# thomaspingel/neilpy

Hardware: AMD Instinct MI355X
Metric: Mcells/s through SMRF progressive_filter, 16384x16384 fp32 DEM (higher is better)
Workload: dtype f32

## Files before the change

### neilpy_amd/csrc/ero_inc_adopt.inc

```
inline constexpr unsigned char kEroIncAdoptF32[65] = {
    0, 0, 0, 0, 0, 0, 0, 0, 0, 0, 0, 0, 0, 0, 0, 0, 0,
    0, 0, 0, 0, 1, 0, 0, 0, 0, 0, 0, 1, 1, 0, 1, 0, 0,
    0, 0, 1, 0, 1, 0, 1, 1, 1, 1, 1, 1, 1, 1, 1, 1, 1,
    0, 0, 0, 0, 0, 0, 0, 0, 0, 0, 0, 0, 0, 0};
```

### neilpy_amd/csrc/morph_incero.h

```cpp
#pragma once
#include "morph_ring.h"

namespace smrf {

#include "ero_inc.inc"
#include "ero_inc_adopt.inc"

#define SMRF_INCERO_MIN_RADIUS 16
#define SMRF_INCERO_MAX_RADIUS 64

template <typename T>
struct IncEroArgs {
  const T* e_prev;
  const T* last;
  T* out;
  int rows, cols;
  long long ld;
  int seg;
  int nt;
  int plain_tiles;
};

template <int R>
struct IncEroCfg {
  static constexpr int N = kEroInc[R].n;
  static constexpr int DY = kEroInc[R].reach;
  static constexpr int TW = 256, NP = 4, ROWS = 2 * NP;
  static constexpr int W = TW + 2 * DY;
  static constexpr int NPOS = (W + TW - 1) / TW;
  static constexpr int NACC = 2 * DY + ROWS;
  static constexpr int G = 4;
  static constexpr int NJ = NP * N;
  static constexpr int NG = (NJ + G - 1) / G;
  static constexpr int gsize(int g) { const int n = NJ - g * G; return n < 0 ? 0 : n > G ? G : n; }
  static constexpr int dy(int k) { return kEroInc[R].p[k].dy; }
  static constexpr int dx(int k) { return kEroInc[R].p[k].dx; }
  static constexpr int slot(int j) { return 2 * (j / N) - dy(j % N) + DY; }
  struct Plan { short seq[NJ > 0 ? NJ : 1], first[NACC]; };
  static constexpr Plan make_plan() {
    Plan pl{};
    int n = 0;
    for (int s = 0; s < NACC; ++s) {
      pl.first[s] = NJ;
      for (int j = 0; j < NJ; ++j)
        if (slot(j) == s) pl.seq[n++] = (short)j;
    }
    for (int i = NJ - 1; i >= 0; --i) pl.first[slot(pl.seq[i])] = pl.first[slot(pl.seq[i]) + 1] = (short)i;
    return pl;
  }
  static constexpr Plan plan = make_plan();
  static constexpr bool plan_ok() {
    int seen[NJ > 0 ? NJ : 1] = {};
    for (int i = 0; i < NJ; ++i) ++seen[plan.seq[i]];
    for (int j = 0; j < NJ; ++j)
      if (seen[j] != 1) return false;
    for (int s = 0; s < NACC; ++s) {
      int firsts = 0, touches = 0;
      for (int i = 0; i < NJ; ++i)
        for (int h = 0; h < 2; ++h)
          if (slot(plan.seq[i]) + h == s) { ++touches; firsts += plan.first[s] == i; }
      if (firsts != (touches > 0)) return false;
      if (s + ROWS < NACC && plan.first[s] < NJ && plan.first[s + ROWS] < NJ && plan.first[s] >= plan.first[s + ROWS]) return false;
    }
    return true;
  }
  static constexpr int DELTA = (ROWS - (2 * DY) % ROWS) % ROWS;
  static constexpr int LDS_CELLS = N > 0 ? 2 * NP * W : 1;
};

template <typename T, int R>
__global__ __launch_bounds__(256) void inc_erode_kernel(const IncEroArgs<T> a) {
  using C = IncEroCfg<R>;
  using T2 = typename Vec2<T>::type;
  constexpr int N = C::N, DY = C::DY, TW = C::TW, NP = C::NP, ROWS = C::ROWS, W = C::W, NPOS = C::NPOS, NACC = C::NACC, G = C::G;
  __shared__ T2 L[C::LDS_CELLS];
  const int tid = threadIdx.x;
  int bx, by;
  smrf_xcd_tile(a.plain_tiles, [] { return true; }, bx, by);
  const int x0 = bx * TW, x = x0 + tid;
  const int ys = by * a.seg, ye = min(a.rows, ys + a.seg);
  if (ys >= ye) return;
  const int xc = x < a.cols ? x : a.cols - 1;
  const int xl = smrf_fold(xc - 1, a.cols), xr = smrf_fold(xc + 1, a.cols);
  int cpos[NPOS];
  bool act[NPOS];
#pragma unroll
  for (int i = 0; i < NPOS; ++i) {
    act[i] = tid + i * TW < W;
    cpos[i] = smrf_fold(x0 - DY + tid + (act[i] ? i * TW : 0), a.cols);
  }
  T acc[NACC];
#pragma unroll
  for (int i = 0; i < NACC; ++i) acc[i] = ident<T>(false);

  static_assert(C::plan_ok(), "the batch plan");
  int o0 = ys - 2 * DY - C::DELTA;
  const int nb = (ye - o0 + ROWS - 1) / ROWS;
  RowFold rf(o0 + DY, a.rows);
  T2 pf[NP][NPOS];
  auto prefetch = [&]() {
#pragma unroll
    for (int p = 0; p < NP; ++p) {
      const T* ra = a.last + (long long)rf.at(2 * p) * a.ld;
      const T* rb = a.last + (long long)rf.at(2 * p + 1) * a.ld;
#pragma unroll
      for (int i = 0; i < NPOS; ++i)
        { pf[p][i].x = ra[cpos[i]]; pf[p][i].y = rb[cpos[i]]; }
    }
    rf.advance(ROWS);
  };
  if constexpr (N > 0) prefetch();

  T outv[ROWS];
  auto store_rows = [&](int ob) {
#pragma unroll
    for (int j = 0; j < ROWS; ++j)
      if (ob + j < ye && x < a.cols) smrf_store_out(a.out + (long long)(ob + j) * a.ld + x, outv[j], a.nt);
  };
  for (int b = 0; b < nb; ++b, o0 += ROWS) {
    const unsigned lds_b = (unsigned)(size_t)(__attribute__((address_space(3))) void*)(L + (b & 1) * NP * W + tid);
    if constexpr (N > 0) {
#pragma unroll
      for (int p = 0; p < NP; ++p)
#pragma unroll
        for (int i = 0; i < NPOS; ++i)
          lds_write2(lds_b + (unsigned)((p * W + (i < NPOS - 1 || act[i] ? i * TW : 0)) * (int)sizeof(T2)), pf[p][i]);
      lds_wait<0>();
      __syncthreads();
    }
    if (o0 - ROWS >= ys) store_rows(o0 - ROWS);
    const bool store = o0 >= ys;
    T ec[ROWS + 2], el[ROWS], er[ROWS];
    if (store) {
      RowFold rfe(o0 - 1, a.rows);
#pragma unroll
      for (int j = 0; j < ROWS + 2; ++j) {
        const T* row = a.e_prev + (long long)rfe.at(j) * a.ld;
        ec[j] = row[xc];
        if (j >= 1 && j <= ROWS) { el[j - 1] = row[xl]; er[j - 1] = row[xr]; }
      }
    }
    if constexpr (N > 0) {
      __builtin_amdgcn_sched_barrier(0);
      prefetch();
      __builtin_amdgcn_sched_barrier(0);
      T old[NACC];
#pragma unroll
      for (int s = 0; s < NACC; ++s) old[s] = acc[s];
      [&]<int... S>(std::integer_sequence<int, S...>) {
        (([&] {
           if constexpr (C::plan.first[S] == C::NJ) acc[S] = S + ROWS < NACC ? old[S + ROWS] : ident<T>(false);
         }()),
         ...);
      }(std::make_integer_sequence<int, NACC>{});
      T2 rd[2 * G][2];
      auto issue = [&]<int I>(std::integral_constant<int, I>) {
        constexpr int J = C::plan.seq[I], p = J / N, k = J % N;
        constexpr int offl = (p * W + DY - C::dx(k)) * (int)sizeof(T2), offr = (p * W + DY + C::dx(k)) * (int)sizeof(T2);
        rd[I % (2 * G)][0] = lds_read2<offl>(lds_b, T());
        rd[I % (2 * G)][1] = lds_read2<offr>(lds_b, T());
      };
      auto update = [&]<int S, int I>(std::integral_constant<int, S>, std::integral_constant<int, I>, const T& l, const T& r) {
        static_assert(S >= 0 && S < NACC, "slot outside the ring");
        if constexpr (C::plan.first[S] != I) op3_acc<false>(acc[S], l, r);
        else if constexpr (S + ROWS < NACC) acc[S] = op3<false>(old[S + ROWS], l, r);
        else acc[S] = op2<false>(l, r);
      };
      auto apply = [&]<int I>(std::integral_constant<int, I> i) {
        constexpr int s = C::slot(C::plan.seq[I]);
        update(std::integral_constant<int, s>{}, i, rd[I % (2 * G)][0].x, rd[I % (2 * G)][1].x);
        update(std::integral_constant<int, s + 1>{}, i, rd[I % (2 * G)][0].y, rd[I % (2 * G)][1].y);
      };
      auto issue_group = [&]<int Gi>(std::integral_constant<int, Gi>) {
        [&]<int... I>(std::integer_sequence<int, I...>) {
          (issue(std::integral_constant<int, Gi * G + I>{}), ...);
        }(std::make_integer_sequence<int, C::gsize(Gi)>{});
      };
      auto apply_group = [&]<int Gi>(std::integral_constant<int, Gi>) {
        [&]<int... I>(std::integer_sequence<int, I...>) {
          (apply(std::integral_constant<int, Gi * G + I>{}), ...);
        }(std::make_integer_sequence<int, C::gsize(Gi)>{});
      };
      issue_group(std::integral_constant<int, 0>{});
      [&]<int... Gi>(std::integer_sequence<int, Gi...>) {
        (([&] {
           if constexpr (Gi + 1 < C::NG) {
             issue_group(std::integral_constant<int, Gi + 1>{});
             lds_wait<2 * C::gsize(Gi + 1)>();
           } else {
             lds_wait<0>();
           }
           apply_group(std::integral_constant<int, Gi>{});
         }()),
         ...);
      }(std::make_integer_sequence<int, C::NG>{});
    }
    if (store) {
#pragma unroll
      for (int j = 0; j < ROWS; ++j) {
        T m = op3<false>(ec[j + 1], el[j], er[j]);
        m = op3<false>(m, ec[j], ec[j + 2]);
        if constexpr (N > 0) m = op2<false>(m, acc[j]);
        outv[j] = m;
      }
    }
  }
  if (o0 - ROWS >= ys) store_rows(o0 - ROWS);
}

template <typename T, int R>
int inc_erode_launch(const IncEroArgs<T>& a_in, hipStream_t stream) {
  using C = IncEroCfg<R>;
  constexpr auto kern = inc_erode_kernel<T, R>;
  int resident;
  bool first;
  if (int rc = smrf_resident<kern>(C::TW, 0, resident, first)) return rc;
  if (first && smrf_sw().ring_debug)
    fprintf(stderr, "smrf inc erode: R=%d pairs=%d reach=%d LDS=%zu, %d workgroups/CU resident\n", R, C::N, C::DY,
            C::LDS_CELLS * 2 * sizeof(T), resident);
  IncEroArgs<T> a = a_in;
  const int strips = (a.cols + C::TW - 1) / C::TW;
  a.seg = smrf_seg_len(a.rows, strips, resident, smrf_sw().ring_rounds, 2 * C::DY + C::DELTA, C::ROWS, std::max(32, 4 * C::DY),
                       smrf_sw().seg_rule, a.seg);
  a.plain_tiles = smrf_sw().xcd_remap ? 0 : 1;
  dim3 grid(strips, (a.rows + a.seg - 1) / a.seg);
  hipLaunchKernelGGL(kern, grid, dim3(C::TW), 0, stream, a);
  SMRF_LAUNCH_CHECK();
  return SMRF_OK;
}

}
```

Before: 4132.

## Share LDS reads between mirrored offset pairs in incremental erosion kernel

The incremental erosion kernel now exploits the vertical mirror symmetry of the structuring-element offset table. Each pair of offsets with opposite dy and the same dx reuses one pair of LDS reads to update two accumulator slots, roughly halving LDS read traffic. A compile-time scheduler orders these items so each ring slot's first write follows the right dependency, either splitting pairs or copying old values when no ordering works. Per-radius tables choose the plan kind and whether the cross-shaped neighbourhood global loads move after the LDS phase, and the adoption table enables the incremental path for more radii. The cost is higher compile-time complexity and register pressure from the rescheduled accumulators.

```diff
diff --git a/neilpy_amd/csrc/ero_inc_adopt.inc b/neilpy_amd/csrc/ero_inc_adopt.inc
--- a/neilpy_amd/csrc/ero_inc_adopt.inc
+++ b/neilpy_amd/csrc/ero_inc_adopt.inc
@@ -1,5 +1,5 @@
 inline constexpr unsigned char kEroIncAdoptF32[65] = {
     0, 0, 0, 0, 0, 0, 0, 0, 0, 0, 0, 0, 0, 0, 0, 0, 0,
-    0, 0, 0, 0, 1, 0, 0, 0, 0, 0, 0, 1, 1, 0, 1, 0, 0,
-    0, 0, 1, 0, 1, 0, 1, 1, 1, 1, 1, 1, 1, 1, 1, 1, 1,
+    0, 0, 0, 0, 1, 0, 0, 0, 0, 0, 0, 1, 1, 0, 1, 1, 1,
+    1, 1, 1, 1, 1, 1, 1, 1, 1, 1, 1, 1, 1, 1, 1, 1, 1,
     0, 0, 0, 0, 0, 0, 0, 0, 0, 0, 0, 0, 0, 0};
diff --git a/neilpy_amd/csrc/morph_incero.h b/neilpy_amd/csrc/morph_incero.h
--- a/neilpy_amd/csrc/morph_incero.h
+++ b/neilpy_amd/csrc/morph_incero.h
@@ -8,6 +8,35 @@
 
 #define SMRF_INCERO_MIN_RADIUS 16
 #define SMRF_INCERO_MAX_RADIUS 64
+
+enum { kIncEroPlain = 0, kIncEroMirrorSplit = 1, kIncEroMirrorCopy = 2 };
+inline constexpr unsigned char kIncEroPlanKind[65] = {
+    1, 1, 1, 1, 1, 1, 1, 1, 1, 1, 1, 1, 1, 1, 1, 1, 1,
+    1, 1, 1, 1, 1, 1, 1, 1, 1, 1, 1, 1, 1, 1, 1, 1, 1,
+    1, 1, 1, 1, 1, 1, 1, 1, 1, 1, 2, 2, 1, 1, 1, 1, 1,
+    1, 1, 1, 1, 1, 1, 1, 1, 1, 1, 1, 1, 1, 1};
+inline constexpr unsigned char kIncEroCrossLate[65] = {
+    0, 0, 0, 0, 0, 0, 0, 0, 0, 0, 0, 0, 0, 0, 0, 0, 0,
+    0, 0, 0, 0, 0, 0, 0, 0, 0, 0, 0, 0, 0, 0, 0, 0, 0,
+    0, 0, 0, 0, 0, 1, 0, 0, 0, 0, 1, 1, 0, 0, 0, 1, 1,
+    0, 0, 0, 0, 0, 0, 0, 0, 0, 0, 0, 0, 0, 0};
+#ifndef SMRF_INCERO_MIRROR_GROUP
+#define SMRF_INCERO_MIRROR_GROUP 2
+#endif
+constexpr int inc_ero_plan_kind(int radius) {
+#ifdef SMRF_INCERO_PLAN
+  return SMRF_INCERO_PLAN;
+#else
+  return kIncEroPlanKind[radius];
+#endif
+}
+constexpr bool inc_ero_cross_late(int radius) {
+#ifdef SMRF_INCERO_LATE
+  return SMRF_INCERO_LATE;
+#else
+  return kIncEroCrossLate[radius] != 0;
+#endif
+}
 
 template <typename T>
 struct IncEroArgs {
@@ -29,41 +58,132 @@
   static constexpr int W = TW + 2 * DY;
   static constexpr int NPOS = (W + TW - 1) / TW;
   static constexpr int NACC = 2 * DY + ROWS;
-  static constexpr int G = 4;
+  static constexpr int KIND = N > 0 ? inc_ero_plan_kind(R) : kIncEroPlain;
+  static constexpr int NM = N / 2;
+  static constexpr int G = KIND == kIncEroPlain ? 4 : SMRF_INCERO_MIRROR_GROUP;
   static constexpr int NJ = NP * N;
-  static constexpr int NG = (NJ + G - 1) / G;
-  static constexpr int gsize(int g) { const int n = NJ - g * G; return n < 0 ? 0 : n > G ? G : n; }
   static constexpr int dy(int k) { return kEroInc[R].p[k].dy; }
   static constexpr int dx(int k) { return kEroInc[R].p[k].dx; }
   static constexpr int slot(int j) { return 2 * (j / N) - dy(j % N) + DY; }
-  struct Plan { short seq[NJ > 0 ? NJ : 1], first[NACC]; };
+  static constexpr int mirror(int j) { return (j / N) * N + N - 1 - j % N; }
+  static constexpr bool mirrored() {
+    for (int k = 0; k < N; ++k)
+      if (dy(k) != -dy(N - 1 - k) || dx(k) != dx(N - 1 - k) || dy(k) == 0) return false;
+    return N % 2 == 0;
+  }
+  static constexpr short NONE = 32767;
+  struct Item { short j; bool both; };
+  struct Plan { short n, splits, copies; Item item[NJ > 0 ? NJ : 1]; short first[NACC]; };
   static constexpr Plan make_plan() {
     Plan pl{};
-    int n = 0;
-    for (int s = 0; s < NACC; ++s) {
-      pl.first[s] = NJ;
-      for (int j = 0; j < NJ; ++j)
-        if (slot(j) == s) pl.seq[n++] = (short)j;
-    }
-    for (int i = NJ - 1; i >= 0; --i) pl.first[slot(pl.seq[i])] = pl.first[slot(pl.seq[i]) + 1] = (short)i;
+    for (int s = 0; s < NACC; ++s) pl.first[s] = NONE;
+    auto emit = [&](int j, bool both) {
+      for (int h = 0; h < (both ? 2 : 1); ++h)
+        for (int b = 0; b < 2; ++b) {
+          short& f = pl.first[slot(h ? mirror(j) : j) + b];
+          if (f == NONE) f = pl.n;
+        }
+      pl.item[pl.n++] = Item{(short)j, both};
+    };
+    if constexpr (KIND == kIncEroPlain) {
+      for (int s = 0; s < NACC; ++s)
+        for (int j = 0; j < NJ; ++j)
+          if (slot(j) == s) emit(j, false);
+    } else {
+      constexpr int NGR = NP * NM;
+      auto jlo = [](int g) { return (g / NM) * N + NM + g % NM; };
+      auto lo = [&](int g) { return slot(jlo(g)); };
+      auto hi = [&](int g) { return slot(mirror(jlo(g))); };
+      bool touched[NACC] = {}, done[NACC] = {};
+      unsigned char state[NGR > 0 ? NGR : 1] = {};
+      for (int g = 0; g < NGR; ++g) touched[lo(g)] = touched[lo(g) + 1] = touched[hi(g)] = touched[hi(g) + 1] = true;
+      auto unready = [&](int g, int part) {
+        int u = 0;
+        for (int h = 0; h < 2; ++h)
+          if (part >> h & 1)
+            for (int b = 0; b < 2; ++b) {
+              const int t = (h ? hi(g) : lo(g)) + b;
+              u += !(done[t] || t < ROWS || !touched[t - ROWS] || done[t - ROWS]);
+            }
+        return u;
+      };
+      auto run = [&](int g, int part) {
+        pl.copies += (short)unready(g, part);
+        if (part & 1) done[lo(g)] = done[lo(g) + 1] = true;
+        if (part & 2) done[hi(g)] = done[hi(g) + 1] = true;
+        state[g] |= (unsigned char)part;
+        emit(part == 2 ? mirror(jlo(g)) : jlo(g), part == 3);
+      };
+      for (int left = 2 * NGR; left > 0;) {
+        int bg = -1, bpart = 0, bkey = 0;
+        for (int g = 0; g < NGR; ++g) {
+          const int part = 3 & ~state[g];
+          if (!part || unready(g, part)) continue;
+          const int key = part & 1 ? lo(g) : hi(g);
+          if (bg < 0 || key < bkey) bg = g, bpart = part, bkey = key;
+        }
+        if (bg < 0 && KIND == kIncEroMirrorSplit) {
+          int bcnt = -1;
+          for (int g = 0; g < NGR; ++g)
+            for (int part = 1; part <= 2 && !state[g]; ++part) {
+              if (unready(g, part)) continue;
+              const int s = part == 1 ? lo(g) : hi(g);
+              const bool was[2] = {done[s], done[s + 1]};
+              done[s] = done[s + 1] = true;
+              state[g] |= (unsigned char)part;
+              int cnt = 0;
+              for (int h = 0; h < NGR; ++h) {
+                const int rest = 3 & ~state[h];
+                const int a = lo(h) - s - ROWS, c = hi(h) - s - ROWS;
+                if (rest && ((a >= -1 && a <= 1) || (c >= -1 && c <= 1)) && !unready(h, rest)) ++cnt;
+              }
+              state[g] = 0;
+              done[s] = was[0], done[s + 1] = was[1];
+              if (cnt > bcnt || (cnt == bcnt && s < bkey)) bg = g, bpart = part, bkey = s, bcnt = cnt;
+            }
+          ++pl.splits;
+        } else if (bg < 0) {
+          int bu = 0;
+          for (int g = 0; g < NGR; ++g) {
+            if (state[g]) continue;
+            const int u = unready(g, 3);
+            if (bg < 0 || u < bu || (u == bu && lo(g) < bkey)) bg = g, bpart = 3, bkey = lo(g), bu = u;
+          }
+        }
+        run(bg, bpart);
+        left -= bpart == 3 ? 2 : 1;
+      }
+    }
     return pl;
   }
   static constexpr Plan plan = make_plan();
+  static constexpr int NI = plan.n;
+  static constexpr int NG = (NI + G - 1) / G;
+  static constexpr int gsize(int g) { const int n = NI - g * G; return n < 0 ? 0 : n > G ? G : n; }
   static constexpr bool plan_ok() {
+    if (N > 0 && !mirrored()) return false;
     int seen[NJ > 0 ? NJ : 1] = {};
-    for (int i = 0; i < NJ; ++i) ++seen[plan.seq[i]];
+    for (int i = 0; i < NI; ++i) {
+      ++seen[plan.item[i].j];
+      if (plan.item[i].both) ++seen[mirror(plan.item[i].j)];
+    }
     for (int j = 0; j < NJ; ++j)
       if (seen[j] != 1) return false;
+    if (KIND == kIncEroPlain ? NI != NJ || plan.splits || plan.copies : NI != NP * NM + plan.splits) return false;
+    if ((KIND == kIncEroMirrorSplit && plan.copies) || (KIND == kIncEroMirrorCopy && plan.splits)) return false;
+    int late = 0;
     for (int s = 0; s < NACC; ++s) {
-      int firsts = 0, touches = 0;
-      for (int i = 0; i < NJ; ++i)
-        for (int h = 0; h < 2; ++h)
-          if (slot(plan.seq[i]) + h == s) { ++touches; firsts += plan.first[s] == i; }
-      if (firsts != (touches > 0)) return false;
-      if (s + ROWS < NACC && plan.first[s] < NJ && plan.first[s + ROWS] < NJ && plan.first[s] >= plan.first[s + ROWS]) return false;
-    }
-    return true;
-  }
+      int earliest = NONE, touches = 0;
+      for (int i = NI - 1; i >= 0; --i)
+        for (int h = 0; h < (plan.item[i].both ? 2 : 1); ++h)
+          for (int b = 0; b < 2; ++b)
+            if (slot(h ? mirror(plan.item[i].j) : plan.item[i].j) + b == s) { ++touches; earliest = i; }
+      if (plan.first[s] != earliest) return false;
+      if (touches && s + ROWS < NACC && plan.first[s + ROWS] != NONE && plan.first[s] >= plan.first[s + ROWS]) ++late;
+    }
+    return late == plan.copies;
+  }
+  static constexpr bool LATE = N > 0 && inc_ero_cross_late(R);
   static constexpr int DELTA = (ROWS - (2 * DY) % ROWS) % ROWS;
   static constexpr int LDS_CELLS = N > 0 ? 2 * NP * W : 1;
 };
@@ -131,7 +251,7 @@
     if (o0 - ROWS >= ys) store_rows(o0 - ROWS);
     const bool store = o0 >= ys;
     T ec[ROWS + 2], el[ROWS], er[ROWS];
-    if (store) {
+    auto cross_loads = [&]() {
       RowFold rfe(o0 - 1, a.rows);
 #pragma unroll
       for (int j = 0; j < ROWS + 2; ++j) {
@@ -139,7 +259,9 @@
         ec[j] = row[xc];
         if (j >= 1 && j <= ROWS) { el[j - 1] = row[xl]; er[j - 1] = row[xr]; }
       }
-    }
+    };
+    if constexpr (!C::LATE)
+      if (store) cross_loads();
     if constexpr (N > 0) {
       __builtin_amdgcn_sched_barrier(0);
       prefetch();
@@ -149,13 +271,13 @@
       for (int s = 0; s < NACC; ++s) old[s] = acc[s];
       [&]<int... S>(std::integer_sequence<int, S...>) {
         (([&] {
-           if constexpr (C::plan.first[S] == C::NJ) acc[S] = S + ROWS < NACC ? old[S + ROWS] : ident<T>(false);
+           if constexpr (C::plan.first[S] == C::NONE) acc[S] = S + ROWS < NACC ? old[S + ROWS] : ident<T>(false);
          }()),
          ...);
       }(std::make_integer_sequence<int, NACC>{});
       T2 rd[2 * G][2];
       auto issue = [&]<int I>(std::integral_constant<int, I>) {
-        constexpr int J = C::plan.seq[I], p = J / N, k = J % N;
+        constexpr int J = C::plan.item[I].j, p = J / N, k = J % N;
         constexpr int offl = (p * W + DY - C::dx(k)) * (int)sizeof(T2), offr = (p * W + DY + C::dx(k)) * (int)sizeof(T2);
         rd[I % (2 * G)][0] = lds_read2<offl>(lds_b, T());
         rd[I % (2 * G)][1] = lds_read2<offr>(lds_b, T());
@@ -167,9 +289,11 @@
         else acc[S] = op2<false>(l, r);
       };
       auto apply = [&]<int I>(std::integral_constant<int, I> i) {
-        constexpr int s = C::slot(C::plan.seq[I]);
+        constexpr int s = C::slot(C::plan.item[I].j), m = C::slot(C::mirror(C::plan.item[I].j));
         update(std::integral_constant<int, s>{}, i, rd[I % (2 * G)][0].x, rd[I % (2 * G)][1].x);
+        if constexpr (C::plan.item[I].both) update(std::integral_constant<int, m>{}, i, rd[I % (2 * G)][0].x, rd[I % (2 * G)][1].x);
         update(std::integral_constant<int, s + 1>{}, i, rd[I % (2 * G)][0].y, rd[I % (2 * G)][1].y);
+        if constexpr (C::plan.item[I].both) update(std::integral_constant<int, m + 1>{}, i, rd[I % (2 * G)][0].y, rd[I % (2 * G)][1].y);
       };
       auto issue_group = [&]<int Gi>(std::integral_constant<int, Gi>) {
         [&]<int... I>(std::integer_sequence<int, I...>) {
@@ -196,6 +320,7 @@
       }(std::make_integer_sequence<int, C::NG>{});
     }
     if (store) {
+      if constexpr (C::LATE) cross_loads();
 #pragma unroll
       for (int j = 0; j < ROWS; ++j) {
         T m = op3<false>(ec[j + 1], el[j], er[j]);
```

Measured after the change: 4245, median of 6. 1.03x the previous value.
